# Chemical118/TREW

Hardware: AMD Instinct MI355X
Metric: Gbases/s scanned (short 5 32, 150 bp reads) (higher is better)
Workload: dtype u32

## Files before the change

### include/trew_hip.h

```cpp
#ifndef TREW_HIP_H
#define TREW_HIP_H

#include <stddef.h>
#include <stdint.h>

#ifdef __cplusplus
extern "C" {
#endif

#define TREW_HIP_ABI_VERSION 4

enum {
    TREW_MODE_SHORT = 0,
    TREW_MODE_PAIR = 1,
    TREW_MODE_LONG = 2,
    TREW_MODE_SEGMENT = 3
};

enum {
    TREW_TABLE_FORWARD_HIGH = 0,
    TREW_TABLE_FORWARD_LOW = 1,
    TREW_TABLE_BACKWARD_HIGH = 2,
    TREW_TABLE_BACKWARD_LOW = 3,
    TREW_TABLE_BOTH_HIGH = 4,
    TREW_TABLE_BOTH_LOW = 5,
    TREW_NUM_TABLES = 6
};

enum {
    TREW_FLAG_NO_FILTER = 1,
    TREW_FLAG_DEBUG_NO_EMIT = 2,
    TREW_FLAG_DEBUG_NO_KLOOP = 4,
    TREW_FLAG_DEBUG_POISON_LDS = 32,
    TREW_FLAG_DEBUG_WIDE_NO_WAIT = 128,
    TREW_FLAG_NO_TIMING = 64,
    TREW_FLAG_COMPAT_G1 = 512,
    TREW_FLAG_DEBUG_NO_JOINT = 2048,
    TREW_FLAG_DEBUG_NO_UNI_DRAIN = 4096,
    TREW_FLAG_DEBUG_NO_GROUP = 1024,
    TREW_FLAG_DEBUG_ANNOT_GENERAL = 8192,
    TREW_FLAG_TRACK_PRESSURE = 256
};

typedef struct {
    int32_t min_mer;
    int32_t max_mer;
    double low_baseline;
    double high_baseline;
    int32_t slice_length;
    int32_t mode;
    int32_t device;
    int32_t n_slots;
    uint64_t max_batch_words;
    uint64_t max_batch_reads;
    uint32_t table_log2_slots;
    uint32_t flags;
    uint64_t max_batch_ascii_bytes;
} trew_hip_params;

typedef struct {
    const uint32_t *words;
    uint64_t n_words;
    const uint32_t *offsets;
// ... 219 lines not shown
```

### trew_amd/__init__.py

```python
from . import capi
from .capi import (
    FLAG_NO_FILTER,
    FLAG_DEBUG_ANNOT_GENERAL,
    FLAG_DEBUG_POISON_LDS,
    FLAG_NO_TIMING,
    FLAG_TRACK_PRESSURE,
    FLAG_COMPAT_G1,
    FLAG_DEBUG_NO_GROUP,
    FLAG_DEBUG_NO_JOINT,
    FLAG_DEBUG_NO_UNI_DRAIN,
    FLAG_DEBUG_WIDE_NO_WAIT,
    MODE_LONG,
    MODE_PAIR,
    MODE_SEGMENT,
    MODE_SHORT,
    TABLE_NAMES,
    TrewHip,
    TrewHipError,
    align,
    annotate,
    chain,
    intervals,
    k_mer_check,
    pack_reads,
    periods,
    refine,
    repeats,
    satellites,
    tandems,
    tracts,
    variants,
)
```

### trew_amd/capi.py

```python
from __future__ import annotations

import ctypes as C
import os

import numpy as np

_HERE = os.path.dirname(os.path.abspath(__file__))
LIB_PATH = os.environ.get("TREW_HIP_LIB") or os.path.join(_HERE, "lib", "libtrew_hip.so")

MODE_SHORT, MODE_PAIR, MODE_LONG, MODE_SEGMENT = 0, 1, 2, 3
FLAG_NO_FILTER = 1
FLAG_DEBUG_POISON_LDS = 32
FLAG_NO_TIMING = 64
FLAG_COMPAT_G1 = 512
FLAG_TRACK_PRESSURE = 256
FLAG_DEBUG_NO_JOINT = 2048
FLAG_DEBUG_NO_UNI_DRAIN = 4096
FLAG_DEBUG_NO_GROUP = 1024
FLAG_DEBUG_ANNOT_GENERAL = 8192
FLAG_DEBUG_WIDE_NO_WAIT = 128
TABLE_NAMES = ("forward_high", "forward_low", "backward_high", "backward_low", "both_high", "both_low")

EXPORTED_SYMBOLS = (
    "trew_hip_init", "trew_hip_destroy", "trew_hip_last_error", "trew_hip_submit", "trew_hip_wait",
    "trew_hip_collect", "trew_hip_reset_tables", "trew_hip_add_rows", "trew_hip_segment_results",
    "trew_hip_filter_masks", "trew_hip_last_timing", "trew_pack_words", "trew_pack_reads",
    "trew_synth_short_ascii", "trew_synth_short_device", "trew_synth_pair_ascii", "trew_synth_pair_device",
    "trew_hip_malloc", "trew_hip_free", "trew_hip_memcpy_h2d", "trew_hip_memcpy_d2h", "trew_hip_abi_version",
    "trew_pack_pairs", "trew_hip_host_alloc", "trew_hip_host_free", "trew_hip_device_count",
    "trew_synth_long_lengths", "trew_synth_long_ascii", "trew_synth_long_device",
    "trew_hip_collect_device", "trew_hip_add_rows_device", "trew_hip_merge", "trew_hip_table_pressure",
    "trew_hip_add_gathered_device", "trew_hip_collect_slice_device", "trew_hip_debug_counters", "trew_hip_debug_worklist", "trew_hip_submit_ascii", "trew_hip_pack_ascii",
    "trew_motif_parse", "trew_hip_annotate", "trew_hip_annotate_results", "trew_annotate_host",
    "trew_hip_tracts", "trew_hip_tracts_results", "trew_tracts_host",
    "trew_hip_intervals", "trew_hip_intervals_results", "trew_intervals_host",
    "trew_hip_variants", "trew_hip_variants_results", "trew_variants_host",
    "trew_hip_periods", "trew_hip_periods_results", "trew_periods_host",
    "trew_hip_chain", "trew_hip_chain_results", "trew_chain_host",
    "trew_hip_repeats", "trew_hip_repeats_results", "trew_repeats_host",
    "trew_hip_satellites", "trew_hip_satellites_results", "trew_satellites_host",
    "trew_hip_align", "trew_hip_align_results", "trew_align_host",
    "trew_hip_refine", "trew_hip_refine_results", "trew_refine_host",
# ... 1103 lines not shown
```

### trew_amd/csrc/kernels/decide_group.inc

```

#define TREW_REGION_LIST(X) \
    X(chunk) X(stage) X(group_setup) X(bounds) X(group) X(dg_loop) X(dg_pick) X(dg_eval) X(er_gaps) X(er_runs) X(er_canon) X(er_merge) X(er_max) \
    X(dg_decision) X(dg_end) X(routing) X(records) X(target) X(target_rows) X(target_eval) X(target_emit) X(fallback)
#define TREW_REGION_ENUM(n) kRegion_##n,
enum { TREW_REGION_LIST(TREW_REGION_ENUM) kRegionCount };
#ifdef TREW_REGION_COUNTS
__device__ unsigned long long g_region[64];
#define TREW_MARK(n)                                                                   \
    do {                                                                               \
        asm volatile("; MARK " #n);                                                    \
        if (lane_id() == 0) atomicAdd(&g_region[kRegion_##n], 1ull);                   \
    } while (0)
#else
#define TREW_MARK(n) asm volatile("; MARK " #n)
#endif
__device__ __forceinline__ void lds_sync() {
    __builtin_amdgcn_fence(__ATOMIC_RELEASE, "wavefront");
    __builtin_amdgcn_wave_barrier();
    __builtin_amdgcn_fence(__ATOMIC_ACQUIRE, "wavefront");
}
#define TREW_DPP(v, ctrl) ((u32) __builtin_amdgcn_update_dpp(0, (int) (v), (ctrl), 0xf, 0xf, false))
__device__ __forceinline__ u32 swap16(u32 v) { return (u32) __builtin_amdgcn_ds_swizzle((int) v, 0x401F); }
template <int G = 16>
__device__ __forceinline__ u32 row_or(u32 v) {
// ... 442 lines not shown
                load_planes_lds<1>(rr, 32u * l, lo1, hi1, nm1);
                nmv = nm1[0] | ~low_mask<true>((int) L - 32 * (int) l);
                const u32 lq = lo1[0] & ~nmv, hq = hi1[0] & ~nmv;
                sq = spread32(__brev(lq)) | (spread32(__brev(hq)) << 1);
            }
            seq[l] = sq;
            nmk[l] = nmv;
        }
    }
    lds_sync();
}

template <typename WT>
__device__ __forceinline__ WT strand_canon(WT w, int k) {
    const WT rc = min_rotation<WT>(revcomp(w, k), k);
    return rc < w ? rc : w;
}

template <typename WT>
__device__ __forceinline__ WT strand_flip(WT w, int k) {
    return min_rotation<WT>(revcomp(w, k), k);
}

template <int NW, typename WT>
__device__ void run_short_group(ExactSmem sm, const DevParams &P, TableRef T, const ReadRef rdA, const ReadRef rdB, bool haveB) {
    const u32 lane = lane_id();
#if defined(TREW_AB_SKIP) && TREW_AB_SKIP >= 5
    return;
#endif
    TREW_MARK(stage);
    PH_T0(t_stage);
    stage_two(sm, rdA, rdB, haveB);
    PH_ADD(PH_STAGE, t_stage);
#if defined(TREW_AB_SKIP) && TREW_AB_SKIP >= 4
    return;
#endif
    TREW_MARK(group_setup);
    const u32 g = lane >> 4, j = lane & 15u;
    const bool second = g >= 2u;
    const u32 is_right = g & 1u;
    ReadRef rd;
    rd.w = second ? rdB.w : rdA.w;
    rd.len = second ? rdB.len : rdA.len;
    rd.nw = second ? rdB.nw : rdA.nw;
    const Segment sg = get_segment(TREW_MODE_SHORT, (int) is_right, rd.len, 0, P.min_mer, P.max_mer, P.slice_len);
    const bool rowvalid = sg.valid && (!second || haveB);
    TREW_MARK(bounds);
    PH_T0(t_bounds);
    lds_sync();
    row_prepare<NW>(sm, rd, sg, rowvalid);
    lds_sync();
    RowSeg<NW> rs;
    row_load<NW>(sm, (int) sg.len, rs);
    u32 bnd0;
    if (P.min_mer + 15 < 32)
        bnd0 = rowvalid ? bound_at_k<NW, true>(rs, (int) sg.len, P.min_mer + (int) j, P.max_mer, P) : 0u;
    else
        bnd0 = rowvalid ? bound_at_k<NW, false>(rs, (int) sg.len, P.min_mer + (int) j, P.max_mer, P) : 0u;
    const u32 bnd1 = rowvalid ? bound_at_k<NW>(rs, (int) sg.len, P.min_mer + 16 + (int) j, P.max_mer, P) : 0u;
#if defined(TREW_AB_SKIP) && TREW_AB_SKIP >= 3
    asm volatile("" ::"v"(bnd0), "v"(bnd1));
    return;
#endif
    PH_ADD(PH_BOUNDS, t_bounds);
    TREW_MARK(group);
    const GroupOut<WT> o = decide_group<NW, WT, false>(sm, P, rs, bnd0, bnd1, second ? 1u : 0u, sg, rowvalid);
#if defined(TREW_AB_SKIP) && TREW_AB_SKIP >= 2
    asm volatile("" ::"v"(o.kk), "v"(o.saved), "v"(o.kept_cnt), "v"((u32) o.kept_canon), "v"((u32) (o.kept_canon >> 32)), "v"((u32) o.punt));
    return;
#endif
    TREW_MARK(routing);
    PH_T0(t_route);
    const u32 mine = rowvalid ? (o.kk | (o.punt ? 1u << 16 : 0u)) : 0u;
    const u32 other = lane_gather(mine, lane ^ 16u);
    const u32 kkL = is_right ? other : mine, kkR = is_right ? mine : other;
    const u32 lkh = kkL & 255u, lkl = (kkL >> 8) & 255u, rkh = kkR & 255u, rkl = (kkR >> 8) & 255u;
    const u32 left_found = (lkh | lkl) != 0u ? 1u : 0u;
    const u32 tgt_h = left_found & (lkh == rkh ? 1u : 0u) & (lkh != 0u ? 1u : 0u);
    const u32 tgt_l = left_found & (lkl == rkl ? 1u : 0u) & (lkl != 0u ? 1u : 0u);
    const u32 myk = o.saved & 255u, items = (o.saved >> 8) & 255u;
    u32 need_old = ((kkL | kkR) >> 16) & 1u;
    u32 rec_mask = 0;
// ... 138 lines not shown
```

### trew_amd/csrc/kernels/exact_kernel.inc

```

#ifndef TREW_EXACT_SHORT_WAVES
#define TREW_EXACT_SHORT_WAVES 5
#endif
#ifndef TREW_EXACT_PAIR_WAVES
#define TREW_EXACT_PAIR_WAVES 4
#endif
#ifndef TREW_EXACT_LONG_WAVES
#define TREW_EXACT_LONG_WAVES 4
#endif
template <int NW, int MODE>
constexpr int exact_waves(bool narrow) {
    return NW >= 10 ? 4
                    : (narrow && NW > 0 && MODE == TREW_MODE_SHORT
                           ? TREW_EXACT_SHORT_WAVES
                           : (narrow && NW > 0 && MODE == TREW_MODE_PAIR ? TREW_EXACT_PAIR_WAVES : (narrow && NW == 5 && MODE == TREW_MODE_LONG ? TREW_EXACT_LONG_WAVES : 6)));
}
template <int NW, int MODE, typename WT>
__global__ __launch_bounds__(64, (exact_waves<NW, MODE>(sizeof(WT) == 8))) void exact_kernel(DevParams P, DevBatch B, DevTableG1 TG, const u32 *wl,
                                                   u32 *wl_count, u32 *wl_count_next, u32 wl_cap, SegResults R, u32 cap, u32 rawwords) {
    struct KernArgs {
        DevParams P;
        DevBatch B;
        DevTableG1 TG;
    };
    static_assert(alignof(DevParams) == 8 && alignof(DevBatch) == 8 && alignof(DevTableG1) == 8, "kernarg layout: 8-byte aligned argument structs");
    static_assert(sizeof(DevParams) % 8 == 0 && sizeof(DevBatch) % 8 == 0, "kernarg layout: no padding between the argument structs");
    static_assert(offsetof(KernArgs, TG) == sizeof(DevParams) + sizeof(DevBatch), "kernarg layout: TG follows P and B");
    static_assert(offsetof(DevTableG1, t) == 0, "TableRef points at DevTableG1::t");
    const TableRef T = (TableRef) ((const char *) __builtin_amdgcn_kernarg_segment_ptr() + offsetof(KernArgs, TG));
#ifdef TREW_AB_EXACT_PRIO
    __builtin_amdgcn_s_setprio(TREW_AB_EXACT_PRIO);
#endif
    if (blockIdx.x == 0 && wl_count_next) {
        for (u32 i = lane_id(); i < (1u + 8u) * 32u; i += 64u) wl_count_next[i] = 0u;
    }
    ExactSmem sm;
    sm.lds = lds_offset_in_kernel();
    sm.cap = cap;
    sm.rawwords = rawwords;
    sm.s0 = 0;
    sm.rs = sm.rnw = 0;
    sm.rw = nullptr;
    u32 n = wl_count[0];
    n = n < wl_cap ? n : wl_cap;
#ifdef TREW_PHASE_PROFILE
    if (lane_id() < 32) ph_lds()[lane_id()] = 0;
    __syncthreads();
// ... 105 lines not shown
        while (cur != ~0ull) {
            TREW_MARK(chunk);
            const u32 nit = chunk_items(cur);
            u32 *const meta = meta_base + bf * kMetaWords;
            PH_T0(t_p0);
            const u64 nxt = resolve_claim();
            PH_ADD(PH_STAGE, t_p0);
            const u32 nxt_nit = nxt != ~0ull ? chunk_items(nxt) : 0u;
            if (nxt_nit) fetch_units(bf ^ 1u, nxt, nxt_nit);
            const u32 hook = nit < kUnits / 2u ? nit : kUnits / 2u;
            PH_CNT(PH_N_READS, nit);
            auto item = [&](u32 t, ReadRef &rd, u32 &unit, bool &staged) __attribute__((always_inline)) {
                rd.len = rfl(meta[4 + t]);
                rd.nw = (rd.len + 31u) >> 5;
                unit = rfl(meta[t / kPer]);
                const u64 off = ((u64) rfl(meta[12 + t]) << 32) | rfl(meta[8 + t]);
                staged = rfl(meta[16 + t]) != 0u;
                rd.w = staged ? (const u32 *) (raw_base + (bf * kChunk + t) * sm.rawwords) : B.words + off;
            };
            ReadRef held;
            held.w = nullptr;
            held.len = held.nw = 0;
            bool have_held = false;
            for (u32 t = 0; t <= nit; t++) {
                if (t == hook && nxt_nit) {
                    PH_T0(t_p1);
                    landed();
                    PH_ADD(PH_STAGE, t_p1);
                    fetch_words(bf ^ 1u, nxt_nit);
                    issue_claim();
                }
                if constexpr (MODE == TREW_MODE_PAIR) {
                    if (t < nit) {
                        ReadRef r0, r1;
                        u32 unit = 0, unit1 = 0;
                        bool st0, st1;
                        item(2u * t, r0, unit, st0);
                        item(2u * t + 1u, r1, unit1, st1);
                        run_pair<NW, WT>(sm, P, T, unit, r0, r1);
                        __syncthreads();
                    }
                    continue;
                }
                ReadRef rd;
                rd.w = nullptr;
                rd.len = rd.nw = 0;
                u32 unit = 0;
                bool ok = false;
                if (t < nit) {
                    bool staged;
                    item(t, rd, unit, staged);
                    ok = grouped && staged && 4 * P.min_mer <= (int) rd.len;
                    if (!ok) {
                        if (MODE == TREW_MODE_SHORT)
                            run_short<NW, WT>(sm, P, T, rd);
                        else
                            run_segment<NW, WT>(sm, P, T, unit, rd, R);
                        __syncthreads();
                        continue;
                    }
                }
                if constexpr (kGroup) {
                    if (ok && !have_held) {
                        held = rd;
                        have_held = true;
                    } else if (have_held) {
                        ReadRef second = held;
                        if (ok) second = rd;
                        run_short_group<NW, WT>(sm, P, T, held, second, ok);
                        have_held = false;
                    }
                }
            }
            PH_T0(t_p2);
            if (nxt_nit) landed();
            PH_ADD(PH_STAGE, t_p2);
            cur = nxt;
            bf ^= 1u;
        }
    } else if (MODE == TREW_MODE_LONG && sizeof(WT) == 8 && NW == 5 && use_group) {
        if constexpr (MODE == TREW_MODE_LONG && sizeof(WT) == 8 && NW == 5) run_long_groups<NW, WT>(sm, P, B, T, wl, heads, n);
    } else {
        for (u32 attempt = 0; attempt < kShards; attempt++) {
            const u32 sh = (my + attempt) & (kShards - 1);
            for (;;) {
                u32 c = 0;
                if (lane == 0) c = atomicAdd(&heads[sh * kHeadStride], 1u);
                c = rfl(c);
                const u64 w0l = ((u64) c * kShards + sh) * kChunk;
                if (w0l >= n) break;
                const u32 w0 = (u32) w0l;
                const u32 nit = (w0 + kChunk < n ? w0 + kChunk : n) - w0;
// ... 52 lines not shown
```

### trew_amd/csrc/trew_capi.cpp

```cpp
#include <hip/hip_runtime.h>

#include <algorithm>
#include <atomic>
#include <cmath>
#include <cstdio>
#include <cstdlib>
#include <cstring>
#include <mutex>
#include <string>
#include <thread>
#include <vector>

#include "trew_common.hpp"
#include "trew_launch.hpp"
#include "trew_measures_host.hpp"
#include "trew_synth.hpp"

using namespace trew;

namespace {

enum Measure { kAnnotate, kTracts, kIntervals, kVariants, kPeriods, kChain, kRepeats, kSatellites, kAlign, kRefine, kTandems, kMeasures };
const char *const kMeasureName[kMeasures] = {"annotate", "tracts", "intervals", "variants", "periods", "chain", "repeats", "satellites", "align", "refine", "tandems"};
struct DevBuf {
// ... 1 lines not shown
    u64 bytes = 0;
};
struct MeasureState {
    DevBuf records;
    DevBuf counts;
    unsigned long long *counter = nullptr;
    unsigned long long *hist = nullptr;
    hipEvent_t ev[2] = {nullptr, nullptr};
    bool valid = false, timed = false;
    u64 n = 0;
    u64 max_log = 0;
    u64 n_counts = 0;
    int n_motifs = 0;
    u32 k[kAnnotMaxMotifs] = {};
};

struct Slot {
    hipStream_t stream = nullptr;
    u32 *d_buf = nullptr;
    u32 *d_words = nullptr, *d_offsets = nullptr, *d_lengths = nullptr;
    unsigned char *d_ascii = nullptr;
    u32 *d_wl = nullptr;
    u32 *d_wl_count = nullptr;
    int2 *d_thr = nullptr;
    int2 *h_thr = nullptr;
    hipEvent_t ev_tail = nullptr, ev_copied = nullptr;
    u32 *h_seen = nullptr;
    u32 thr_length = 0;
    SegResults res = {nullptr, nullptr, nullptr, nullptr};
    static constexpr int kRing = 128;
    hipEvent_t ev[kRing][3] = {};
    u64 n_launches = 0;
    u64 n_submits = 0;
    u64 n_reported = 0;
    u64 n_units = 0;
    AnnotMotifDev *d_motifs = nullptr, *h_motifs = nullptr;
    int motifs_staged = 0;
    MeasureState measure[kMeasures];
};

thread_local std::string g_init_error;
thread_local std::string g_thread_error;
constexpr size_t kWlCountWords = 32 + 8 * 32;
constexpr size_t kWlCountBytes = kWlCountWords * 4;

}
// ... 203 lines not shown
    if ((e = hipEventCreateWithFlags(&ctx->ev_producer, hipEventDisableTiming)) != hipSuccess) return bail("hipEventCreate", e);
    ctx->slots.resize((size_t) p.n_slots);
    for (auto &s : ctx->slots) {
        if ((e = hipStreamCreateWithFlags(&s.stream, hipStreamNonBlocking)) != hipSuccess) return bail("hipStreamCreate", e);
        if ((e = hipEventCreateWithFlags(&s.ev_tail, hipEventDisableTiming)) != hipSuccess) return bail("hipEventCreate", e);
        if ((e = hipEventCreateWithFlags(&s.ev_copied, hipEventDisableTiming)) != hipSuccess) return bail("hipEventCreate", e);
        {
            const size_t words = 2 * (size_t) p.max_batch_reads + (size_t) p.max_batch_words + 8;
            if ((e = hipMalloc((void **) &s.d_buf, words * 4)) != hipSuccess) return bail("hipMalloc(batch buffer)", e);
            if ((e = hipMemsetAsync(s.d_buf, 0, words * 4, ctx->fill_stream)) != hipSuccess) return bail("hipMemsetAsync", e);
            s.d_offsets = s.d_buf;
            s.d_lengths = s.d_buf + p.max_batch_reads;
            s.d_words = s.d_buf + 2 * (size_t) p.max_batch_reads;
        }
        if (p.max_batch_ascii_bytes) {
            if ((e = hipMalloc((void **) &s.d_ascii, p.max_batch_ascii_bytes + 256)) != hipSuccess) return bail("hipMalloc(text buffer)", e);
            if ((e = hipMemsetAsync(s.d_ascii, 0, p.max_batch_ascii_bytes + 256, ctx->fill_stream)) != hipSuccess) return bail("hipMemsetAsync", e);
        }
        if ((e = hipMalloc((void **) &s.d_thr, kThrTableBytes)) != hipSuccess) return bail("hipMalloc(thresholds)", e);
        if ((e = hipHostMalloc((void **) &s.h_thr, kThrTableBytes + kDiagWords * 4, hipHostMallocDefault)) != hipSuccess) return bail("hipHostMalloc(thresholds)", e);
        s.h_seen = (u32 *) ((char *) s.h_thr + kThrTableBytes);
        memset(s.h_seen, 0, kDiagWords * 4);
        if ((e = hipMalloc((void **) &s.d_wl, p.max_batch_reads * sizeof(u32))) != hipSuccess) return bail("hipMalloc(worklist)", e);
        if ((e = hipMalloc((void **) &s.d_wl_count, 2 * kWlCountBytes)) != hipSuccess) return bail("hipMalloc(wl_count)", e);
        if ((e = hipMemsetAsync(s.d_wl_count, 0, 2 * kWlCountBytes, ctx->fill_stream)) != hipSuccess) return bail("hipMemsetAsync", e);
        if (p.mode == TREW_MODE_SEGMENT) {
            if ((e = hipMalloc((void **) &s.res.k_high, p.max_batch_reads * 4)) != hipSuccess) return bail("hipMalloc", e);
            if ((e = hipMalloc((void **) &s.res.k_low, p.max_batch_reads * 4)) != hipSuccess) return bail("hipMalloc", e);
            if ((e = hipMalloc((void **) &s.res.seq_high, p.max_batch_reads * 8)) != hipSuccess) return bail("hipMalloc", e);
            if ((e = hipMalloc((void **) &s.res.seq_low, p.max_batch_reads * 8)) != hipSuccess) return bail("hipMalloc", e);
            if ((e = hipMalloc((void **) &s.res.seq_high_hi, p.max_batch_reads * 8)) != hipSuccess) return bail("hipMalloc", e);
            if ((e = hipMalloc((void **) &s.res.seq_low_hi, p.max_batch_reads * 8)) != hipSuccess) return bail("hipMalloc", e);
        }
        for (int i = 0; i < Slot::kRing; i++)
            for (int j = 0; j < 3; j++)
                if ((e = hipEventCreate(&s.ev[i][j])) != hipSuccess) return bail("hipEventCreate", e);
    }
    if (int rc = order_behind_fills(ctx)) {
        g_init_error = g_thread_error;
        trew_hip_destroy(ctx);
        return rc;
    }
    *out = ctx;
    return 0;
}

extern "C" void trew_hip_destroy(trew_hip_ctx *ctx) {
    if (!ctx) return;
    (void) hipSetDevice(ctx->p.device);
    for (auto &s : ctx->slots) {
        if (s.stream) (void) hipStreamSynchronize(s.stream);
        if (s.d_buf) (void) hipFree(s.d_buf);
        if (s.d_ascii) (void) hipFree(s.d_ascii);
        if (s.d_thr) (void) hipFree(s.d_thr);
        if (s.h_thr) (void) hipHostFree(s.h_thr);
        if (s.d_wl) (void) hipFree(s.d_wl);
        if (s.d_wl_count) (void) hipFree(s.d_wl_count);
        if (s.res.k_high) (void) hipFree(s.res.k_high);
        if (s.res.k_low) (void) hipFree(s.res.k_low);
        if (s.res.seq_high) (void) hipFree(s.res.seq_high);
        if (s.res.seq_low) (void) hipFree(s.res.seq_low);
        if (s.res.seq_high_hi) (void) hipFree(s.res.seq_high_hi);
        if (s.res.seq_low_hi) (void) hipFree(s.res.seq_low_hi);
        for (int i = 0; i < Slot::kRing; i++)
            for (int j = 0; j < 3; j++)
                if (s.ev[i][j]) (void) hipEventDestroy(s.ev[i][j]);
        if (s.d_motifs) (void) hipFree(s.d_motifs);
        if (s.h_motifs) (void) hipHostFree(s.h_motifs);
        for (auto &st : s.measure) {
            for (void *p : {st.records.p, st.counts.p, (void *) st.counter, (void *) st.hist})
                if (p) (void) hipFree(p);
            for (auto e : st.ev)
                if (e) (void) hipEventDestroy(e);
        }
        if (s.ev_tail) (void) hipEventDestroy(s.ev_tail);
        if (s.ev_copied) (void) hipEventDestroy(s.ev_copied);
        if (s.stream) (void) hipStreamDestroy(s.stream);
    }
    if (ctx->copy_stream) (void) hipStreamSynchronize(ctx->copy_stream);
// ... 209 lines not shown
            g_thread_error = std::string(#expr) + ": " + hipGetErrorString(e_);               \
            return submit_failed((int) e_);                                                    \
        }                                                                                      \
    } while (0)
    const int2 *d_thr = nullptr;
    if (int rc = stage_thresholds(ctx, s, db, &d_thr)) return submit_failed(rc);
    const bool compat_g1 = (ctx->p.flags & TREW_FLAG_COMPAT_G1) != 0;
    if (compat_g1) SUBMIT_CHK(hipMemsetAsync(ctx->g1.pair_flags, 0, db.n_units, s.stream));
    const bool timed = !(ctx->p.flags & TREW_FLAG_NO_TIMING);
    hipEvent_t *ev = s.ev[s.n_submits % Slot::kRing];
    if (timed) SUBMIT_CHK(hipEventRecord(ev[0], s.stream));
    SUBMIT_CHK(launch_filter(s.stream, (u32) ctx->n_cu, max_seg, ctx->dp, db, s.d_wl, wl_count, wl_cap, nullptr, 0, ctx->table.overflow, d_thr));
    if (timed) SUBMIT_CHK(hipEventRecord(ev[1], s.stream));
    const u32 exact_seg = ctx->p.mode == TREW_MODE_LONG ? std::min<u32>(max_len, (u32) (2 * ctx->dp.slice_len - 1)) : max_len;
    const u32 cap = std::max<u32>(64u, ((exact_seg + 1 + 63u) / 64u) * 64u);
    const u32 rawwords = ctx->p.mode == TREW_MODE_LONG ? 4u : 3u * ((max_len + 31u) / 32u) + 1u;
    const int me = (int) (&s - ctx->slots.data());
    const int prev = ctx->last_slot.exchange(me, std::memory_order_relaxed);
    bool share = false;
    if (prev >= 0 && prev != me) {
        share = hipStreamQuery(ctx->slots[(size_t) prev].stream) == hipErrorNotReady;
        (void) hipGetLastError();
    }
    SUBMIT_CHK(launch_exact(s.stream, (u32) ctx->n_cu, db.n_units, ctx->dp, db, ctx->table_g1, s.d_wl, wl_count, wl_count_next, wl_cap, s.res, cap, rawwords, max_seg, share));
    if (timed) SUBMIT_CHK(hipEventRecord(ev[2], s.stream));
    if (compat_g1) {
        SUBMIT_CHK(launch_g1_apply(s.stream, ctx->table, ctx->g1, db, ctx->dp.min_mer, ctx->g1_carry[ctx->g1_batches & 1], ctx->g1_carry[(ctx->g1_batches + 1) & 1],
                                   ctx->g1_carry_cap));
        ctx->g1_batches++;
    }
#undef SUBMIT_CHK
    s.n_launches++;
    s.n_submits++;
    if (ctx->p.flags & TREW_FLAG_TRACK_PRESSURE)
        HIPCHK(ctx, hipMemcpyAsync(s.h_seen, ctx->table.overflow, kDiagWords * 4, hipMemcpyDeviceToHost, s.stream));
    return 0;
}

extern "C" int trew_hip_submit(trew_hip_ctx *ctx, const trew_hip_batch *batch, int slot) {
    if (!ctx || !batch) return -1;
    if (slot < 0 || slot >= (int) ctx->slots.size()) return fail(ctx, "slot out of range");
    HIPCHK(ctx, hipSetDevice(ctx->p.device));
    Slot &s = ctx->slots[(size_t) slot];
    u32 max_seg = 0, max_len = 0;
    if (int rc = batch_geometry(ctx, batch, &max_seg, &max_len)) return rc;
    DevBatch db;
    if (int rc = stage_batch(ctx, batch, s, &db)) return rc;
// ... 1408 lines not shown
```

### trew_amd/csrc/trew_kernels.hip

```cpp
#include <hip/hip_runtime.h>

#include <algorithm>
#include <cstdlib>

#include "trew_common.hpp"
#include "trew_launch.hpp"
#include "trew_synth.hpp"

#ifndef TREW_FILTER_THREADS
#define TREW_FILTER_THREADS 256
#endif

namespace trew {

typedef unsigned __int128 u128;

#include "kernels/helpers.inc"
#include "kernels/bound.inc"
#include "kernels/prefilter.inc"
#include "kernels/count_table.inc"
#include "kernels/exact_core.inc"
#include "kernels/decide_group.inc"
#include "kernels/driver_long.inc"
#include "kernels/driver_pair.inc"
#include "kernels/exact_kernel.inc"
#include "kernels/g1_compat.inc"
#include "kernels/table_kernels.inc"
#include "kernels/synth_kernels.inc"
#include "kernels/annotate.inc"
#include "kernels/tracts.inc"
#include "kernels/intervals.inc"
#include "kernels/variants.inc"
#include "kernels/periods.inc"
#include "kernels/chain.inc"
#include "kernels/repeats.inc"
#include "kernels/satellites.inc"
#include "kernels/align.inc"
#include "kernels/refine.inc"
#include "kernels/tandems.inc"

int pick_nw(u32 max_seg_len) {
    if (max_seg_len <= 95) return 3;
    if (max_seg_len <= 159) return 5;
    if (max_seg_len <= 319) return 10;
    return 32;
// ... 72 lines not shown
    u64 blocks = (B.n_units + threads - 1) / threads;
    const u64 persistent = (u64) n_cu * (u64) per_cu;
    if (blocks > persistent) blocks = persistent;
    hipLaunchKernelGGL(fn, dim3((u32) blocks), dim3(threads), 0, st, P, B, wl, wl_count, wl_cap, dbg_masks, dbg_slots, max_seg, diag, d_thr);
    return hipGetLastError();
}

hipError_t fallback_counters_read(u32 *out) { return hipMemcpyFromSymbol(out, HIP_SYMBOL(g_fallback), sizeof(u32) * kFallbackWords); }
hipError_t fallback_counters_clear(hipStream_t st) {
    void *p = nullptr;
    const hipError_t e = hipGetSymbolAddress(&p, HIP_SYMBOL(g_fallback));
    return e != hipSuccess ? e : hipMemsetAsync(p, 0, sizeof(u32) * kFallbackWords, st);
}

u32 exact_lds_bytes_host(u32 cap, u32 rawwords, u32 wordbytes) { return exact_lds_bytes(cap, rawwords, wordbytes); }

hipError_t launch_g1_apply(hipStream_t st, const DevTable &T, const DevG1 &G, const DevBatch &B, int min_mer, const trew_hip_row *carry_in,
                           trew_hip_row *carry_out, u32 carry_cap) {
    hipLaunchKernelGGL(g1_apply_kernel, dim3(256), dim3(256), 0, st, T, G, B, min_mer, carry_in, carry_out, carry_cap);
    hipLaunchKernelGGL(g1_finish_kernel, dim3(1), dim3(1), 0, st, G);
    return hipGetLastError();
}

hipError_t launch_exact(hipStream_t st, u32 n_cu, u64 n_units, const DevParams &P, const DevBatch &B, const DevTableG1 &T,
                        const u32 *wl, u32 *wl_count, u32 *wl_count_next, u32 wl_cap, const SegResults &R, u32 cap, u32 rawwords,
                        u32 max_seg_len, bool share) {
    const bool wide = P.max_mer > 32;
    const u32 lds = exact_lds_bytes(cap, rawwords, wide ? 16u : 8u);
    const u32 bound_len = P.mode == TREW_MODE_LONG ? (u32) P.slice_len : max_seg_len;
    const int nw = (P.flags & TREW_FLAG_NO_FILTER) ? 0 : pick_nw(bound_len);
    typedef void (*kern_t)(DevParams, DevBatch, DevTableG1, const u32 *, u32 *, u32 *, u32, SegResults, u32, u32);
    kern_t fn = nullptr;
#define TREW_PICK_MODE(NWV, WTV)                                                      \
    switch (P.mode) {                                                                 \
    case TREW_MODE_SHORT: fn = exact_kernel<NWV, TREW_MODE_SHORT, WTV>; break;        \
    case TREW_MODE_PAIR: fn = exact_kernel<NWV, TREW_MODE_PAIR, WTV>; break;          \
    case TREW_MODE_LONG: fn = exact_kernel<NWV, TREW_MODE_LONG, WTV>; break;          \
    default: fn = exact_kernel<NWV, TREW_MODE_SEGMENT, WTV>; break;                   \
    }
    if (!wide) {
        switch (nw) {
        case 3: TREW_PICK_MODE(3, u64) break;
        case 5: TREW_PICK_MODE(5, u64) break;
        case 10: TREW_PICK_MODE(10, u64) break;
        default: TREW_PICK_MODE(0, u64) break;
        }
    } else {
        switch (nw) {
        case 3: TREW_PICK_MODE(3, u128) break;
        case 5: TREW_PICK_MODE(5, u128) break;
        case 10: TREW_PICK_MODE(10, u128) break;
        default: TREW_PICK_MODE(0, u128) break;
        }
    }
#undef TREW_PICK_MODE
    static thread_local kern_t cached_fn = nullptr;
    static thread_local u32 cached_lds = 0;
    static thread_local int cached_per_cu = 0;
    int per_cu = 8;
    if (cached_fn == fn && cached_lds == lds) {
        per_cu = cached_per_cu;
    } else {
        if (hipOccupancyMaxActiveBlocksPerMultiprocessor(&per_cu, (const void *) fn, 64, lds) != hipSuccess || per_cu < 1) per_cu = 8;
        cached_fn = fn;
        cached_lds = lds;
        cached_per_cu = per_cu;
    }
    per_cu = per_cu > 32 ? 32 : per_cu;
    if (share && P.mode == TREW_MODE_SHORT) per_cu = std::max(1, per_cu / 2);
    if (const char *e = getenv("TREW_EXACT_WAVES_PER_CU")) per_cu = std::max(1, atoi(e));
    const u64 full = (u64) n_cu * (u64) per_cu;
    const u32 grid = (u32) std::min<u64>(full, std::max<u64>(n_units / 16, 64));
    hipLaunchKernelGGL(fn, dim3(grid), dim3(64), lds, st, P, B, T, wl, wl_count, wl_count_next, wl_cap, R, cap, rawwords);
    return hipGetLastError();
}

hipError_t launch_add_rows(hipStream_t st, const DevTable &T, const trew_hip_row *d_rows, u64 n, u32 *d_flags) {
    if (n == 0) return hipSuccess;
    const dim3 grid((u32) ((n + 255) / 256));
    if (d_flags) hipLaunchKernelGGL(table_check_rows_kernel, grid, dim3(256), 0, st, d_rows, n, d_flags);
    hipLaunchKernelGGL(table_add_rows_kernel, grid, dim3(256), 0, st, T, d_rows, n, (const u32 *) d_flags);
    return hipGetLastError();
}

hipError_t launch_add_gathered(hipStream_t st, const DevTable &T, const trew_hip_row *d_buf, u32 n_slices, u32 own, u64 slice_rows, u32 *d_flags) {
    const u64 total = (u64) n_slices * (slice_rows + 1ull);
    if (total == 0) return hipSuccess;
    const dim3 grid((u32) ((total + 255) / 256));
    hipLaunchKernelGGL(table_check_gathered_kernel, grid, dim3(256), 0, st, d_buf, n_slices, own, slice_rows, d_flags);
    hipLaunchKernelGGL(table_add_gathered_kernel, grid, dim3(256), 0, st, T, d_buf, n_slices, own, slice_rows, (const u32 *) d_flags);
    return hipGetLastError();
}

hipError_t launch_pack_ascii(hipStream_t st, const unsigned char *d_bases, const u32 *d_byte_offsets, const u32 *d_lengths, const u32 *d_word_offsets,
                             u32 uniform_length, u64 n_reads, u64 n_triples, u32 *d_words) {
    if (n_triples == 0) return hipSuccess;
// ... 131 lines not shown
```

### trew_amd/csrc/trew_launch.hpp

```cpp
#pragma once
#include <hip/hip_runtime.h>

#include "trew_common.hpp"

namespace trew {

int pick_nw(u32 max_seg_len);

hipError_t launch_filter(hipStream_t st, u32 n_cu, u32 max_seg_len, const DevParams &P, const DevBatch &B, u32 *wl, u32 *wl_count,
                         u32 wl_cap, u64 *dbg_masks, int dbg_slots, u32 *diag, const int2 *d_thr);
void fill_thresholds(const DevParams &P, u32 uniform_length, int2 *table);
hipError_t launch_exact(hipStream_t st, u32 n_cu, u64 n_units, const DevParams &P, const DevBatch &B, const DevTableG1 &T,
                        const u32 *wl, u32 *wl_count, u32 *wl_count_next, u32 wl_cap, const SegResults &R, u32 cap, u32 rawwords,
                        u32 max_seg_len, bool share);
u32 exact_lds_bytes_host(u32 cap, u32 rawwords, u32 wordbytes);
hipError_t launch_g1_apply(hipStream_t st, const DevTable &T, const DevG1 &G, const DevBatch &B, int min_mer, const trew_hip_row *carry_in,
                           trew_hip_row *carry_out, u32 carry_cap);
hipError_t fallback_counters_read(u32 *out);
hipError_t fallback_counters_clear(hipStream_t st);
hipError_t launch_add_rows(hipStream_t st, const DevTable &T, const trew_hip_row *d_rows, u64 n, u32 *d_flags);
hipError_t launch_add_gathered(hipStream_t st, const DevTable &T, const trew_hip_row *d_buf, u32 n_slices, u32 own, u64 slice_rows, u32 *d_flags);
hipError_t launch_pack_ascii(hipStream_t st, const unsigned char *d_bases, const u32 *d_byte_offsets, const u32 *d_lengths, const u32 *d_word_offsets,
                             u32 uniform_length, u64 n_reads, u64 n_triples, u32 *d_words);
hipError_t launch_compact(hipStream_t st, const DevTable &T, u64 n_slots, u32 wide_log2_slots, int table, trew_hip_row *d_rows, u64 cap,
                          unsigned long long *d_n);
hipError_t launch_slice_finish(hipStream_t st, trew_hip_row *d_slice, u64 slice_rows, const unsigned long long *d_n, const trew_hip_row *d_spill_rows,
                               const u32 *d_spill_n, u32 spill_cap);
hipError_t launch_annotate(hipStream_t st, u32 n_cu, const DevBatch &B, const AnnotMotifDev *d_motifs, int n_motifs, u32 max_len, bool general,
                           trew_hip_annot *d_out);
hipError_t launch_tracts(hipStream_t st, u32 n_cu, const DevBatch &B, const AnnotMotifDev *d_motifs, int n_motifs, int penalty, trew_hip_tract *d_out);
hipError_t launch_intervals(hipStream_t st, u32 n_cu, const DevBatch &B, const AnnotMotifDev *d_motifs, int n_motifs, const IntervalRulesDev &rules,
                            const IntervalLog &lg, u32 *d_counts);
hipError_t launch_variants(hipStream_t st, u32 n_cu, const DevBatch &B, const AnnotMotifDev *d_motifs, int n_motifs, trew_hip_variant *d_out,
                           unsigned long long *d_hist, unsigned long long *d_reads_with);
hipError_t launch_periods(hipStream_t st, u32 n_cu, const DevBatch &B, int min_period, int max_period, int penalty, u32 min_score, trew_hip_period *d_out);
hipError_t launch_chain(hipStream_t st, u32 n_cu, const DevBatch &B, const AnnotMotifDev *d_motifs, int n_motifs, const ChainLog &lg, u32 *d_counts);
hipError_t launch_repeats(hipStream_t st, u32 n_cu, const DevBatch &B, int min_period, int max_period, int penalty, u32 min_score, const RepeatLog &lg,
// ... 13 lines not shown
```

Measured before the change: 2089.

## Precompute per-k bound words in a separate bounds kernel before exact pass

Adds a bounds_kernel that computes the per-k filter bound words for each read half and writes them to a device buffer. The grouped short-read path then loads these precomputed bounds instead of running row_prepare, its LDS syncs and bound_at_k inside the exact kernel. This moves the bound computation into a lane-per-half kernel with better occupancy and takes it off the LDS-heavy exact kernel. The cost is an extra launch and a global round trip for the bound buffer, which only covers up to bnd_cap worklist positions; reads past that fall back to the old in-kernel computation.

Result: faster. 2112, median of 6 (+1.1%).

```diff
diff --git a/include/trew_hip.h b/include/trew_hip.h
--- a/include/trew_hip.h
+++ b/include/trew_hip.h
@@ -39,6 +39,7 @@
     TREW_FLAG_DEBUG_NO_UNI_DRAIN = 4096,
     TREW_FLAG_DEBUG_NO_GROUP = 1024,
     TREW_FLAG_DEBUG_ANNOT_GENERAL = 8192,
+    TREW_FLAG_DEBUG_SMALL_BOUNDS = 16384,
     TREW_FLAG_TRACK_PRESSURE = 256
 };
 
diff --git a/trew_amd/__init__.py b/trew_amd/__init__.py
--- a/trew_amd/__init__.py
+++ b/trew_amd/__init__.py
@@ -9,6 +9,7 @@
     FLAG_DEBUG_NO_GROUP,
     FLAG_DEBUG_NO_JOINT,
     FLAG_DEBUG_NO_UNI_DRAIN,
+    FLAG_DEBUG_SMALL_BOUNDS,
     FLAG_DEBUG_WIDE_NO_WAIT,
     MODE_LONG,
     MODE_PAIR,
diff --git a/trew_amd/capi.py b/trew_amd/capi.py
--- a/trew_amd/capi.py
+++ b/trew_amd/capi.py
@@ -18,6 +18,7 @@
 FLAG_DEBUG_NO_UNI_DRAIN = 4096
 FLAG_DEBUG_NO_GROUP = 1024
 FLAG_DEBUG_ANNOT_GENERAL = 8192
+FLAG_DEBUG_SMALL_BOUNDS = 16384
 FLAG_DEBUG_WIDE_NO_WAIT = 128
 TABLE_NAMES = ("forward_high", "forward_low", "backward_high", "backward_low", "both_high", "both_low")
 
diff --git a/trew_amd/csrc/kernels/bounds_pass.inc b/trew_amd/csrc/kernels/bounds_pass.inc
--- /dev/null
+++ b/trew_amd/csrc/kernels/bounds_pass.inc
@@ -0,0 +1,96 @@
+
+constexpr u32 kBoundsTileStride = kBoundWords + 1;
+
+__device__ __forceinline__ u32 pack_bound_word(u32 m8, u32 count, u32 links, u32 has_n, int k, int gmax, const DevParams &P) {
+    const u32 runs = count - links < 127u ? count - links : 127u;
+    const double dm = (double) m8, dc = (double) count;
+    const double tl = P.low * dc, th = P.high * dc;
+    u32 pass_lo = dm > tl ? 1u : 0u, pass_hi = dm > th ? 1u : 0u;
+    const bool amb = fabs(dm - tl) <= 1e-9 || fabs(dm - th) <= 1e-9;
+    if (__any(amb)) {
+        const double ub = count ? dm / dc : 0.0;
+        pass_lo = ub >= P.low ? 1u : 0u;
+        pass_hi = ub >= P.high ? 1u : 0u;
+    }
+    const bool inr = k <= gmax && count != 0u;
+    return inr ? (m8 | (count << 10) | (runs << 20) | (pass_lo << 27) | (pass_hi << 28) | (has_n << 29)) : (has_n << 29);
+}
+
+template <int NW>
+__global__ __launch_bounds__(64) void bounds_kernel(DevParams P, DevBatch B, const u32 *__restrict__ wl, const u32 *__restrict__ wl_count, u32 wl_cap,
+                                                    u32 *__restrict__ bnd, u32 bnd_cap) {
+    static_assert(NW == 3, "the k loop is written for three words: halves of at most 95 bases");
+    __shared__ u32 tile[64 * kBoundsTileStride];
+    const u32 lane = lane_id();
+    u32 n = wl_count[0];
+    n = n < wl_cap ? n : wl_cap;
+    n = n < bnd_cap ? n : bnd_cap;
+    const u64 total = 2ull * n;
+    const int klo = P.min_mer, khi = P.max_mer < P.min_mer + (int) kBoundWords - 1 ? P.max_mer : P.min_mer + (int) kBoundWords - 1;
+    for (u64 base = (u64) blockIdx.x * 64u; base < total; base += (u64) gridDim.x * 64u) {
+        const u64 idx = base + lane;
+        const bool active = idx < total;
+        const u32 half = (u32) idx & 1u;
+        ReadRef rd;
+        rd.w = B.words;
+        rd.len = rd.nw = 0;
+        if (active) rd = get_read(B, wl[idx >> 1]);
+        const Segment sg = get_segment(TREW_MODE_SHORT, (int) half, rd.len, 0, P.min_mer, P.max_mer, P.slice_len);
+        const bool can = active && sg.valid && sg.len <= 32u * NW - 1u;
+        if (!can) rd.nw = 0;
+        const int L = can ? (int) sg.len : 0;
+        u32 lo[3], hi[3], nm[3], V[3], P1[3], P2[3], P3[3];
+        load_planes<3>(rd, sg.start, lo, hi, nm);
+        segment_setup<3, false, true, true>(lo, hi, nm, L, V, P1, P2, P3);
+        const u32 has_n = segment_has_n<3>(nm, L) != 0u ? 1u : 0u;
+        for (int t = 1; t < klo; t++) drain_v_step3(V);
+        const int Lmax = (int) wave_max_u32((u32) L);
+        u32 *const row = tile + lane * kBoundsTileStride;
+        int k = klo;
+        for (const int b = khi < Lmax - 64 ? khi : Lmax - 64; k <= b; k++) {
+            const u32 bs = (u32) k;
+            u32 F1[3], F2[3], F3[3], E[3];
+#pragma unroll
+            for (int j = 0; j < 3; j++) {
+                const int jn = j < 2 ? j + 1 : 0;
+                F1[j] = xor_and(P1[j], alignbit(j < 2 ? P1[jn] : 0u, P1[j], bs), V[j]);
+                F2[j] = xor_and(P2[j], alignbit(j < 2 ? P2[jn] : 0u, P2[j], bs), V[j]);
+                F3[j] = P3[j] ^ alignbit(j < 2 ? P3[jn] : 0u, P3[j], bs);
+                E[j] = ~((lo[j] ^ alignbit(j < 2 ? lo[jn] : 0u, lo[j], bs)) | (hi[j] ^ alignbit(j < 2 ? hi[jn] : 0u, hi[j], bs)));
+            }
+            const u32 count = bcnt_acc(V[2], bcnt_acc(V[1], __popc(V[0])));
+            const u32 m8 = max_bucket8<3>(F1, F2, F3, V, count);
+            row[k - klo] = pack_bound_word(m8, count, class_links<3>(V, E), has_n, k, P.max_mer, P);
+            drain_v_step3(V);
+        }
+        if (k <= khi) {
+            const int o = L > 63 ? L - 63 : 0;
+            const u64 Q1 = container64(P1, o), Q2 = container64(P2, o), Q3 = container64(P3, o), Ql = container64(lo, o), Qh = container64(hi, o);
+            u64 Vq = ((u64) V[1] << 32) | V[0];
+            for (; k <= khi; k++) {
+                const u32 sh = (u32) (k - o);
+                const u64 S1 = Q1 >> sh, S2 = Q2 >> sh, S3 = Q3 >> sh, Sl = Ql >> sh, Sh = Qh >> sh;
+                const u32 Vw[2] = {(u32) Vq, (u32) (Vq >> 32)};
+                const u32 F1[2] = {xor_and(P1[0], (u32) S1, Vw[0]), xor_and(P1[1], (u32) (S1 >> 32), Vw[1])};
+                const u32 F2[2] = {xor_and(P2[0], (u32) S2, Vw[0]), xor_and(P2[1], (u32) (S2 >> 32), Vw[1])};
+                const u32 F3[2] = {P3[0] ^ (u32) S3, P3[1] ^ (u32) (S3 >> 32)};
+                const u32 E[2] = {~((lo[0] ^ (u32) Sl) | (hi[0] ^ (u32) Sh)), ~((lo[1] ^ (u32) (Sl >> 32)) | (hi[1] ^ (u32) (Sh >> 32)))};
+                const u32 count = bcnt_acc(Vw[1], __popc(Vw[0]));
+                const u32 m8 = max_bucket8<2>(F1, F2, F3, Vw, count);
+                row[k - klo] = pack_bound_word(m8, count, class_links<2>(Vw, E), has_n, k, P.max_mer, P);
+                Vq &= Vq >> 1;
+            }
+        }
+        for (int ki = khi >= klo ? khi - klo + 1 : 0; ki < (int) kBoundWords; ki++) row[ki] = has_n << 29;
+        lds_sync();
+        const u64 left = total - base;
+        const u32 words = (left < 64u ? (u32) left : 64u) * kBoundWords;
+        u32 *const dst = bnd + base * kBoundWords;
+#pragma unroll 4
+        for (u32 r = 0; r < kBoundWords; r++) {
+            const u32 w = r * 64u + lane;
+            if (w < words) dst[w] = tile[(w >> 5) * kBoundsTileStride + (w & 31u)];
+        }
+        lds_sync();
+    }
+}
diff --git a/trew_amd/csrc/kernels/decide_group.inc b/trew_amd/csrc/kernels/decide_group.inc
--- a/trew_amd/csrc/kernels/decide_group.inc
+++ b/trew_amd/csrc/kernels/decide_group.inc
@@ -488,12 +488,49 @@
     return min_rotation<WT>(revcomp(w, k), k);
 }
 
-template <int NW, typename WT>
-__device__ void run_short_group(ExactSmem sm, const DevParams &P, TableRef T, const ReadRef rdA, const ReadRef rdB, bool haveB) {
+constexpr u32 kBoundWords = 32;
+constexpr u32 kBoundItemWords = 2 * kBoundWords;
+struct NoStoredBounds {
+    static constexpr bool kAny = false;
+};
+struct StoredBounds {
+    static constexpr bool kAny = true;
+    u32 posA, posB;
+};
+struct ExactKernArgs {
+    DevParams P;
+    DevBatch B;
+    DevTableG1 TG;
+    const u32 *wl;
+    u32 *wl_count, *wl_count_next;
+    u32 wl_cap;
+    SegResults R;
+    u32 cap, rawwords;
+    const u32 *bnd;
+    u32 bnd_cap;
+};
+template <int NW, typename WT, typename SB>
+__device__ void run_short_group(ExactSmem sm, const DevParams &P, TableRef T, const ReadRef rdA, const ReadRef rdB, bool haveB, const SB sb) {
     const u32 lane = lane_id();
 #if defined(TREW_AB_SKIP) && TREW_AB_SKIP >= 5
     return;
 #endif
+    u32 st0 = 0, st1 = 0;
+    bool stored = false;
+    if constexpr (SB::kAny) {
+        typedef const __attribute__((address_space(4))) u64 *c64;
+        typedef const __attribute__((address_space(4))) u32 *c32;
+        const u64 ka = (u64) __builtin_amdgcn_kernarg_segment_ptr();
+        const u32 bcap = *(c32) (ka + offsetof(ExactKernArgs, bnd_cap));
+        const u32 posA = rfl(sb.posA), posB = rfl(sb.posB);
+        stored = posA < bcap && posB < bcap;
+        if (stored && (lane < 32u || haveB)) {
+            const u32 *const base = (const u32 *) *(c64) (ka + offsetof(ExactKernArgs, bnd));
+            const u32 *src = base + ((u64) (lane < 32u ? posA : posB) * 2u + ((lane >> 4) & 1u)) * kBoundWords + (lane & 15u);
+            st0 = src[0];
+            st1 = src[16];
+        }
+    }
     TREW_MARK(stage);
     PH_T0(t_stage);
     stage_two(sm, rdA, rdB, haveB);
@@ -513,17 +550,34 @@
     const bool rowvalid = sg.valid && (!second || haveB);
     TREW_MARK(bounds);
     PH_T0(t_bounds);
-    lds_sync();
-    row_prepare<NW>(sm, rd, sg, rowvalid);
-    lds_sync();
     RowSeg<NW> rs;
-    row_load<NW>(sm, (int) sg.len, rs);
-    u32 bnd0;
-    if (P.min_mer + 15 < 32)
-        bnd0 = rowvalid ? bound_at_k<NW, true>(rs, (int) sg.len, P.min_mer + (int) j, P.max_mer, P) : 0u;
-    else
-        bnd0 = rowvalid ? bound_at_k<NW, false>(rs, (int) sg.len, P.min_mer + (int) j, P.max_mer, P) : 0u;
-    const u32 bnd1 = rowvalid ? bound_at_k<NW>(rs, (int) sg.len, P.min_mer + 16 + (int) j, P.max_mer, P) : 0u;
+    u32 bnd0, bnd1;
+    if (stored) {
+        u32 nm[NW];
+        ReadRef r = rd;
+        if (!rowvalid) r.nw = 0;
+        load_planes_lds<NW>(r, sg.start, rs.lo, rs.hi, nm);
+        u32 anyn = 0;
+#pragma unroll
+        for (int w = 0; w < NW; w++) {
+            rs.v1[w] = ~nm[w] & low_mask((int) sg.len - 32 * w);
+            rs.P1[w] = rs.P2[w] = rs.P3[w] = 0;
+            anyn |= ~rs.v1[w] & low_mask((int) sg.len - 32 * w);
+        }
+        rs.has_n = anyn != 0u ? 1u : 0u;
+        bnd0 = rowvalid ? st0 : 0u;
+        bnd1 = rowvalid ? st1 : 0u;
+    } else {
+        lds_sync();
+        row_prepare<NW>(sm, rd, sg, rowvalid);
+        lds_sync();
+        row_load<NW>(sm, (int) sg.len, rs);
+        if (P.min_mer + 15 < 32)
+            bnd0 = rowvalid ? bound_at_k<NW, true>(rs, (int) sg.len, P.min_mer + (int) j, P.max_mer, P) : 0u;
+        else
+            bnd0 = rowvalid ? bound_at_k<NW, false>(rs, (int) sg.len, P.min_mer + (int) j, P.max_mer, P) : 0u;
+        bnd1 = rowvalid ? bound_at_k<NW>(rs, (int) sg.len, P.min_mer + 16 + (int) j, P.max_mer, P) : 0u;
+    }
 #if defined(TREW_AB_SKIP) && TREW_AB_SKIP >= 3
     asm volatile("" ::"v"(bnd0), "v"(bnd1));
     return;
diff --git a/trew_amd/csrc/kernels/exact_kernel.inc b/trew_amd/csrc/kernels/exact_kernel.inc
--- a/trew_amd/csrc/kernels/exact_kernel.inc
+++ b/trew_amd/csrc/kernels/exact_kernel.inc
@@ -17,12 +17,9 @@
 }
 template <int NW, int MODE, typename WT>
 __global__ __launch_bounds__(64, (exact_waves<NW, MODE>(sizeof(WT) == 8))) void exact_kernel(DevParams P, DevBatch B, DevTableG1 TG, const u32 *wl,
-                                                   u32 *wl_count, u32 *wl_count_next, u32 wl_cap, SegResults R, u32 cap, u32 rawwords) {
-    struct KernArgs {
-        DevParams P;
-        DevBatch B;
-        DevTableG1 TG;
-    };
+                                                   u32 *wl_count, u32 *wl_count_next, u32 wl_cap, SegResults R, u32 cap, u32 rawwords,
+                                                   const u32 *bnd, u32 bnd_cap) {
+    typedef ExactKernArgs KernArgs;
     static_assert(alignof(DevParams) == 8 && alignof(DevBatch) == 8 && alignof(DevTableG1) == 8, "kernarg layout: 8-byte aligned argument structs");
     static_assert(sizeof(DevParams) % 8 == 0 && sizeof(DevBatch) % 8 == 0, "kernarg layout: no padding between the argument structs");
     static_assert(offsetof(KernArgs, TG) == sizeof(DevParams) + sizeof(DevBatch), "kernarg layout: TG follows P and B");
@@ -174,6 +171,7 @@
             held.w = nullptr;
             held.len = held.nw = 0;
             bool have_held = false;
+            u32 held_pos = 0;
             for (u32 t = 0; t <= nit; t++) {
                 if (t == hook && nxt_nit) {
                     PH_T0(t_p1);
@@ -213,13 +211,25 @@
                     }
                 }
                 if constexpr (kGroup) {
+                    const u32 pos = (u32) cur + t;
                     if (ok && !have_held) {
                         held = rd;
+                        held_pos = pos;
                         have_held = true;
                     } else if (have_held) {
                         ReadRef second = held;
                         if (ok) second = rd;
-                        run_short_group<NW, WT>(sm, P, T, held, second, ok);
+                        if constexpr (NW == 3) {
+                            StoredBounds sb;
+                            sb.posA = held_pos;
+                            sb.posB = ok ? pos : held_pos;
+                            ReadRef first = held;
+                            first.nw = (first.len + 31u) >> 5;
+                            second.nw = (second.len + 31u) >> 5;
+                            run_short_group<NW, WT>(sm, P, T, first, second, ok, sb);
+                        } else {
+                            run_short_group<NW, WT>(sm, P, T, held, second, ok, NoStoredBounds());
+                        }
                         have_held = false;
                     }
                 }
diff --git a/trew_amd/csrc/trew_capi.cpp b/trew_amd/csrc/trew_capi.cpp
--- a/trew_amd/csrc/trew_capi.cpp
+++ b/trew_amd/csrc/trew_capi.cpp
@@ -47,6 +47,8 @@
     unsigned char *d_ascii = nullptr;
     u32 *d_wl = nullptr;
     u32 *d_wl_count = nullptr;
+    u32 *d_bnd = nullptr;
+    u32 bnd_cap = 0;
     int2 *d_thr = nullptr;
     int2 *h_thr = nullptr;
     hipEvent_t ev_tail = nullptr, ev_copied = nullptr;
@@ -296,6 +298,11 @@
         s.h_seen = (u32 *) ((char *) s.h_thr + kThrTableBytes);
         memset(s.h_seen, 0, kDiagWords * 4);
         if ((e = hipMalloc((void **) &s.d_wl, p.max_batch_reads * sizeof(u32))) != hipSuccess) return bail("hipMalloc(worklist)", e);
+        if (bounds_pass_applies(ctx->dp, 1)) {
+            const u64 share = std::min<u64>(std::max<u64>(p.max_batch_reads / 32, std::min<u64>(p.max_batch_reads, 1ull << 16)), 1ull << 22);
+            s.bnd_cap = (p.flags & TREW_FLAG_DEBUG_SMALL_BOUNDS) ? 64u : (u32) share;
+            if ((e = hipMalloc((void **) &s.d_bnd, (size_t) s.bnd_cap * bounds_entry_bytes())) != hipSuccess) return bail("hipMalloc(bounds)", e);
+        }
         if ((e = hipMalloc((void **) &s.d_wl_count, 2 * kWlCountBytes)) != hipSuccess) return bail("hipMalloc(wl_count)", e);
         if ((e = hipMemsetAsync(s.d_wl_count, 0, 2 * kWlCountBytes, ctx->fill_stream)) != hipSuccess) return bail("hipMemsetAsync", e);
         if (p.mode == TREW_MODE_SEGMENT) {
@@ -329,6 +336,7 @@
         if (s.d_thr) (void) hipFree(s.d_thr);
         if (s.h_thr) (void) hipHostFree(s.h_thr);
         if (s.d_wl) (void) hipFree(s.d_wl);
+        if (s.d_bnd) (void) hipFree(s.d_bnd);
         if (s.d_wl_count) (void) hipFree(s.d_wl_count);
         if (s.res.k_high) (void) hipFree(s.res.k_high);
         if (s.res.k_low) (void) hipFree(s.res.k_low);
@@ -584,7 +592,10 @@
         share = hipStreamQuery(ctx->slots[(size_t) prev].stream) == hipErrorNotReady;
         (void) hipGetLastError();
     }
-    SUBMIT_CHK(launch_exact(s.stream, (u32) ctx->n_cu, db.n_units, ctx->dp, db, ctx->table_g1, s.d_wl, wl_count, wl_count_next, wl_cap, s.res, cap, rawwords, max_seg, share));
+    const bool with_bounds = s.d_bnd != nullptr && bounds_pass_applies(ctx->dp, max_seg);
+    if (with_bounds) SUBMIT_CHK(launch_bounds(s.stream, (u32) ctx->n_cu, db.n_units, ctx->dp, db, s.d_wl, wl_count, wl_cap, s.d_bnd, s.bnd_cap));
+    SUBMIT_CHK(launch_exact(s.stream, (u32) ctx->n_cu, db.n_units, ctx->dp, db, ctx->table_g1, s.d_wl, wl_count, wl_count_next, wl_cap, s.res, cap, rawwords, max_seg, share,
+                            with_bounds ? s.d_bnd : nullptr, s.bnd_cap));
     if (timed) SUBMIT_CHK(hipEventRecord(ev[2], s.stream));
     if (compat_g1) {
         SUBMIT_CHK(launch_g1_apply(s.stream, ctx->table, ctx->g1, db, ctx->dp.min_mer, ctx->g1_carry[ctx->g1_batches & 1], ctx->g1_carry[(ctx->g1_batches + 1) & 1],
diff --git a/trew_amd/csrc/trew_kernels.hip b/trew_amd/csrc/trew_kernels.hip
--- a/trew_amd/csrc/trew_kernels.hip
+++ b/trew_amd/csrc/trew_kernels.hip
@@ -21,6 +21,7 @@
 #include "kernels/count_table.inc"
 #include "kernels/exact_core.inc"
 #include "kernels/decide_group.inc"
+#include "kernels/bounds_pass.inc"
 #include "kernels/driver_long.inc"
 #include "kernels/driver_pair.inc"
 #include "kernels/exact_kernel.inc"
@@ -139,15 +140,31 @@
     return hipGetLastError();
 }
 
+bool bounds_pass_applies(const DevParams &P, u32 max_seg_len) {
+    return P.mode == TREW_MODE_SHORT && P.max_mer <= 32 && !(P.flags & TREW_FLAG_NO_FILTER) && pick_nw(max_seg_len) == 3 &&
+           P.max_mer - P.min_mer < (int) kBoundWords && !(P.flags & TREW_FLAG_DEBUG_NO_GROUP);
+}
+size_t bounds_entry_bytes() { return kBoundItemWords * sizeof(u32); }
+
+hipError_t launch_bounds(hipStream_t st, u32 n_cu, u64 n_units, const DevParams &P, const DevBatch &B, const u32 *wl, const u32 *wl_count,
+                         u32 wl_cap, u32 *bnd, u32 bnd_cap) {
+    if (n_units == 0 || bnd_cap == 0) return hipSuccess;
+    const u64 most = (std::min<u64>(n_units, bnd_cap) * 2 + 63) / 64;
+    const u32 grid = (u32) std::min<u64>((u64) n_cu * 16ull, most);
+    hipLaunchKernelGGL(bounds_kernel<3>, dim3(grid), dim3(64), 0, st, P, B, wl, wl_count, wl_cap, bnd, bnd_cap);
+    return hipGetLastError();
+}
+
 hipError_t launch_exact(hipStream_t st, u32 n_cu, u64 n_units, const DevParams &P, const DevBatch &B, const DevTableG1 &T,
                         const u32 *wl, u32 *wl_count, u32 *wl_count_next, u32 wl_cap, const SegResults &R, u32 cap, u32 rawwords,
-                        u32 max_seg_len, bool share) {
+                        u32 max_seg_len, bool share, const u32 *bnd, u32 bnd_cap) {
     const bool wide = P.max_mer > 32;
     const u32 lds = exact_lds_bytes(cap, rawwords, wide ? 16u : 8u);
     const u32 bound_len = P.mode == TREW_MODE_LONG ? (u32) P.slice_len : max_seg_len;
     const int nw = (P.flags & TREW_FLAG_NO_FILTER) ? 0 : pick_nw(bound_len);
-    typedef void (*kern_t)(DevParams, DevBatch, DevTableG1, const u32 *, u32 *, u32 *, u32, SegResults, u32, u32);
+    typedef void (*kern_t)(DevParams, DevBatch, DevTableG1, const u32 *, u32 *, u32 *, u32, SegResults, u32, u32, const u32 *, u32);
     kern_t fn = nullptr;
+    if (!bounds_pass_applies(P, max_seg_len)) bnd = nullptr;
 #define TREW_PICK_MODE(NWV, WTV)                                                      \
     switch (P.mode) {                                                                 \
     case TREW_MODE_SHORT: fn = exact_kernel<NWV, TREW_MODE_SHORT, WTV>; break;        \
@@ -188,7 +205,7 @@
     if (const char *e = getenv("TREW_EXACT_WAVES_PER_CU")) per_cu = std::max(1, atoi(e));
     const u64 full = (u64) n_cu * (u64) per_cu;
     const u32 grid = (u32) std::min<u64>(full, std::max<u64>(n_units / 16, 64));
-    hipLaunchKernelGGL(fn, dim3(grid), dim3(64), lds, st, P, B, T, wl, wl_count, wl_count_next, wl_cap, R, cap, rawwords);
+    hipLaunchKernelGGL(fn, dim3(grid), dim3(64), lds, st, P, B, T, wl, wl_count, wl_count_next, wl_cap, R, cap, rawwords, bnd, bnd ? bnd_cap : 0u);
     return hipGetLastError();
 }
 
diff --git a/trew_amd/csrc/trew_launch.hpp b/trew_amd/csrc/trew_launch.hpp
--- a/trew_amd/csrc/trew_launch.hpp
+++ b/trew_amd/csrc/trew_launch.hpp
@@ -12,7 +12,11 @@
 void fill_thresholds(const DevParams &P, u32 uniform_length, int2 *table);
 hipError_t launch_exact(hipStream_t st, u32 n_cu, u64 n_units, const DevParams &P, const DevBatch &B, const DevTableG1 &T,
                         const u32 *wl, u32 *wl_count, u32 *wl_count_next, u32 wl_cap, const SegResults &R, u32 cap, u32 rawwords,
-                        u32 max_seg_len, bool share);
+                        u32 max_seg_len, bool share, const u32 *bnd, u32 bnd_cap);
+bool bounds_pass_applies(const DevParams &P, u32 max_seg_len);
+size_t bounds_entry_bytes();
+hipError_t launch_bounds(hipStream_t st, u32 n_cu, u64 n_units, const DevParams &P, const DevBatch &B, const u32 *wl, const u32 *wl_count,
+                         u32 wl_cap, u32 *bnd, u32 bnd_cap);
 u32 exact_lds_bytes_host(u32 cap, u32 rawwords, u32 wordbytes);
 hipError_t launch_g1_apply(hipStream_t st, const DevTable &T, const DevG1 &G, const DevBatch &B, int min_mer, const trew_hip_row *carry_in,
                            trew_hip_row *carry_out, u32 carry_cap);
```
